# cvxopt/smcp

Hardware: AMD Instinct MI355X
Metric: Newton KKT solves/sec (higher is better)
Workload: dtype f64; 1 GPU; synth50k nested block-arrow SDP n=50000, 8073 cliques, m=100; kktsolver=chol, n=50000, cliques=8073, m=100, blkval_doubles=2493568, update_doubles=10689536, parallelism=single

## Files before the change

### smcp_amd/csrc/capi.hip

```cpp
#include <hip/hip_runtime.h>
#include <memory>
#include <unordered_map>

#include <algorithm>
#include <chrono>
#include <cstdio>
#include <cstring>
#include <map>
#include <new>
#include <string>
#include <cxxabi.h>
#include <cstdlib>
#include <atomic>
#include <thread>
#include <type_traits>
#include <vector>

#include "../../include/smcp_amd.h"
#include "constraints.hpp"
#include "context.hpp"
#include "hostpar.hpp"
#include "switches.hpp"
#include "front_generic.hip"
#include "front_mfma.hip"
// ... 322 lines not shown
      return c->D.info_host[t];
    }
  return 0;
}

constexpr int NT = 256;

template <class F>
void for_levels_up(csp_ctx* c, F f) {
  for (int64_t l = 0; l < c->S.nlev; ++l) {
    int64_t b = c->S.levptr[l], e = c->S.levptr[l + 1];
    f(c->D.levidx + b, (int)(e - b));
  }
}
template <class F>
void for_levels_down(csp_ctx* c, F f) {
  for (int64_t l = c->S.nlev - 1; l >= 0; --l) {
    int64_t b = c->S.levptr[l], e = c->S.levptr[l + 1];
    f(c->D.levidx + b, (int)(e - b));
  }
}

inline unsigned gather_parts(int namax, int64_t pairs = (int64_t)1 << 40, int ncu = 0) {
  const int base = std::max(1, std::min(64, (namax * namax) / (NT * 32)));
  if (pairs * base >= 2 * (int64_t)ncu) return (unsigned)base;
  const int cap = std::max(1, std::min(64, (namax * namax) / (NT * 2)));
  return (unsigned)std::max<int64_t>(base, std::min<int64_t>(cap, (2 * (int64_t)ncu + pairs - 1) / std::max<int64_t>(1, pairs)));
}
inline int namax_of(csp_ctx* c, const int32_t* lev) {
  const int64_t off = lev - c->D.levidx;
  const auto& lp = c->S.levptr;
  const int64_t l = std::upper_bound(lp.begin(), lp.end(), off) - lp.begin() - 1;
  return (l >= 0 && l < (int64_t)c->lev_namax.size()) ? c->lev_namax[l] : 0;
}

void gather_all(csp_ctx* c, const double* x, int64_t ldx, int nrhs, double* updbase, hipStream_t st) {
  TreeArgs a = tree_args(c);
  for_levels_down(c, [&](const int32_t* lev, int cnt) {
    a.lev = lev;
    launch(c, KID_gather_level, k_gather_level, dim3(cnt, nrhs, gather_parts(namax_of(c, lev), (int64_t)cnt * nrhs, c->D.ncu)), dim3(NT), st, a, x, ldx, updbase);
  });
}

int prepare_yaa(csp_ctx* c, const double* Y, bool need_fac, hipStream_t st, bool need_inv = false, bool allow_partial = false);
void complete_fac(csp_ctx* c, hipStream_t st);


constexpr size_t LDS_LIMIT = 160 * 1024 - 2048;

bool cache_off() {
  static int nocache = -1;
  if (nocache < 0) { const char* e = sw_str("SMCP_NOCACHE"); nocache = (e && e[0] == '1') ? 1 : 0; }
  return nocache == 1;
}

bool use_generic(const csp_ctx* c) {
  static int g = -1;
  if (g < 0) { const char* e = sw_str("SMCP_GENERIC"); g = (e && e[0] == '1') ? 1 : 0; }
  return g == 1 || (c && c->deterministic);
}

MfmaArgs mfma_args(csp_ctx* c, const double* ysc, int ymode, int nrhs) {
  MfmaArgs a;
  a.t = tree_args(c);
  a.t.lev = c->D.lev2idx;
  a.LK = c->D.lk;
  a.ysc = ysc;
  a.ymode = ymode;
  a.nnmax = a.namax = 0;
  a.nchmax = a.panmax = a.pkmax = a.plansum = 0;
  a.nrhs = nrhs;
  { static int sk = -1; if (sk < 0) { const char* e = sw_str("SMCP_SKIP"); sk = e ? atoi(e) : 0; } a.skip = sk; }
  a.dbg = (a.skip & 64) ? (unsigned long long*)(c->D.red + 768) : nullptr;
  a.lfd = c->D.lfd;
  a.dn = 0; a.dld = 0;
  a.kc_ptr = nullptr; a.kc_off = nullptr; a.kc_val = nullptr; a.kc_ids = nullptr;
  a.sp_rt = c->D.sp_rt; a.sp_mk = c->D.sp_mk;
  a.kc_stride = 0; a.kc_j0 = 0;
  a.nnmin = 0;
  a.grp_ptr = nullptr; a.grp_list = nullptr; a.chskip = nullptr; a.famt_ngrp = 0;
  a.fz_on = 0; a.fz_nat = 0; a.fz_cnn = 0; a.fz_stride = 0; a.fz_recl = 0;
  a.fz_tab = nullptr; a.fz_no = nullptr; a.fz_slot = nullptr; a.fz_ptr = nullptr; a.fz_pk = nullptr; a.fz_s = nullptr;
  a.level = 0; a.nS = 0; a.famna = a.fampan = a.fampk = a.famcna = a.famnn = a.famcnn = 0;
  return a;
}

int rhs_groups(int ncl, int nrhs, int target) {
  int g = (target + ncl - 1) / ncl;
  return std::max(1, std::min(g, nrhs));
}

template <class F>
void for_level_classes(csp_ctx* c, int64_t l, MfmaArgs a, F f, int set = 0) {
  const LevelClass& L = set ? c->sets[set].lvl[l] : c->lvl[l];
  const int32_t* base = set ? c->sets[set].lev2 + c->sets[set].off[l] : c->D.lev2idx + c->S.levptr[l];
  if (L.nI) {
    a.t.lev = base;
    a.nnmax = L.nnmaxI;
    a.namax = L.namaxI;
    a.nchmax = L.nchmaxI;
    a.panmax = L.panmaxI;
    a.pkmax = L.pkmaxI;
    a.plansum = L.plansumI;
    a.level = (int)l; a.nS = (int)L.nS; a.famna = L.famna; a.fampan = L.fampan; a.fampk = L.fampk; a.famcna = L.famcna; a.famnn = L.famnn; a.famcnn = L.famcnn;
    size_t lds = (size_t)mfma_lds_doubles(L.nnmaxI, L.namaxI) * sizeof(double);
    f(true, a, (int)L.nI, lds, lds > 48 * 1024 ? 512 : 256);
  }
  if (L.nII) {
    a.t.lev = base + L.nI;
    a.level = (int)l;
    a.nnmax = L.nnmaxII;
    a.nnmin = L.nnminII;
    a.namax = L.namaxII;
    a.nchmax = L.nchmaxII;
    f(false, a, (int)L.nII, (size_t)0, 1024);
  }
}


template <class F>
void for_all_large(csp_ctx* c, MfmaArgs a, F f) {
  if (!c->D.nII_total) return;
  a.t.lev = c->D.lev3idx + c->D.nI_total;
  a.nnmax = c->D.nnmaxII_all;
  a.namax = c->D.namaxII_all;
  f(a, (int)c->D.nII_total);
}

bool use_large() {
  static int g = -1;
  if (g < 0) { const char* e = sw_str("SMCP_LARGE"); g = (e && e[0] == '0') ? 0 : 1; }
  return g == 1;
}
inline unsigned umax1(int x) { return (unsigned)std::max(1, x); }
static int fact_threads(const MfmaArgs& am, int thr, int kind) {
  static int t[3] = {0, 0, 0};
  if (!t[0]) {
    auto rd = [](const char* n, int d, int hi) { const char* e = sw_str(n); int v = e ? atoi(e) : d; return (v >= 64 && v <= hi && !(v & 63)) ? v : d; };
    t[0] = rd("SMCP_FTHR_CHOL", 128, 1024); t[1] = rd("SMCP_FTHR_PINV", 256, 1024); t[2] = rd("SMCP_FTHR_YAA", 64, 256);
  }
  if (kind == 2 && am.nnmax <= 16 && am.namax > 32 && am.namax <= 64) {
    static int tm = 0;
    if (!tm) { const char* e = sw_str("SMCP_FTHR_YAA_MID"); tm = e ? atoi(e) : 256; if (tm < 64 || tm > 256 || (tm & 63)) tm = 256; }
    return tm;
  }
  return (am.nnmax <= 16 && am.namax <= 32) ? t[kind] : thr;
}

static bool alds_route(csp_ctx* c, const MfmaArgs& a, int cnt, int nrhs, int& nz, size_t& bytes) {
  static int alds = -1;
  if (alds < 0) { const char* e = sw_str("SMCP_ALDS"); alds = (e && e[0] == '0') ? 0 : 1; }
  const int nfmax = a.nnmax + a.namax;
  static int zenv = -1;
  if (zenv < 0) { const char* e = sw_str("SMCP_ALDS_Z"); zenv = e ? atoi(e) : 0; }
  const int64_t pairs = std::max<int64_t>(1, (int64_t)cnt * nrhs);
  nz = 1;
  if (zenv > 0) nz = zenv;
  else if (a.nchmax >= 256) nz = (int)std::max<int64_t>(1, std::min<int64_t>({(int64_t)a.nchmax / 16, (int64_t)64, (4 * (int64_t)c->D.ncu + pairs - 1) / pairs}));
  else if (nrhs >= 16 && 2 * pairs <= c->D.ncu && a.nchmax >= 32)
    nz = (int)std::max<int64_t>(1, std::min<int64_t>({(int64_t)a.nchmax / 16, (int64_t)8, (2 * (int64_t)c->D.ncu + pairs - 1) / pairs}));
  nz = std::max(1, std::min(nz, std::max(1, a.nchmax)));
  bytes = (size_t)(lf_alds_doubles(nfmax) + 4 * ((a.nchmax + nz - 1) / nz) + 2) * sizeof(double);
  if (!(alds && a.nchmax > 0 && pairs * nz >= 32 && nfmax <= LF_ALDS_MAXNF && bytes <= LDS_LIMIT)) return false;
  static bool attr = false;
  if (!attr) { attr = hipFuncSetAttribute((const void*)k_lf_assemble_lds, hipFuncAttributeMaxDynamicSharedMemorySize, 160 * 1024 - 1024) == hipSuccess; }
  return attr;
// ... 1672 lines not shown
  if (c->scal_lstar < 0) {
    int64_t ls = S.nlev;
    while (ls > 0 && c->lvl[(size_t)ls - 1].nI == 0) --ls;
    c->scal_lstar = ls;
    std::vector<int> lev_of((size_t)S.nsn, 0);
    for (int64_t l = 0; l < S.nlev; ++l)
      for (int64_t q = S.levptr[l]; q < S.levptr[l + 1]; ++q) lev_of[(size_t)S.levidx[q]] = (int)l;
    int64_t t0 = bl;
    for (int64_t k = 0; k < S.nsn; ++k) if (lev_of[(size_t)k] == S.nlev - 1) t0 = std::min<int64_t>(t0, S.blkptr[k]);
    for (int64_t k = 0; k < S.nsn; ++k) if (S.blkptr[k] >= t0 && lev_of[(size_t)k] != S.nlev - 1) { t0 = 0; break; }
    c->scal_tail0 = t0;
  }
  const int64_t lstar = c->scal_lstar;
  const bool fast = !use_generic(c) && use_large() && D.gp_tptr && !cache_off() && Fork::enabled() && scaling_overlap_on() &&
                    c->ntrial == 1 && lstar < S.nlev && (lstar > 0 || D.nI_total == 0) && D.yaa && S.updlen() > 0 && !c->verify_cache;
  if (!fast) {
    const bool li = top_li_whole(c);
    if (li) { D.lk_tag_L = D.lk_tag_Y = nullptr; D.part_valid = false; D.lk_gen++; }
    if (int rc = cholesky_impl(c, L, (void*)st, 0, li)) return rc;
    HIPCHK(hipMemcpyAsync(Y, L, sizeof(double) * bl, hipMemcpyDeviceToDevice, st));
    if (int rc = projected_inverse_impl(c, Y, (void*)st, 0, li)) return rc;
    c->D.lk_tag_L = L;
    if (flags & SCALING_FAC) { if (int rc = prepare_yaa(c, Y, true, st)) return rc; HIPCHK(end_call(c)); }
    return 0;
  }
  invalidate_tags(c, L);
  invalidate_tags(c, Y);
  HIPCHK(zero_flag(c, st));
  const int64_t last = S.nlev - 1;
  const int64_t tail0 = c->scal_tail0;
  MfmaArgs a0 = mfma_args(c, nullptr, 0, 1);
  a0.LK = nullptr;
  TreeArgs t = tree_args(c);
  int nnI = 0;
  for (const LevelClass& Lc : c->lvl) if (Lc.nI) nnI = std::max(nnI, (int)Lc.nnmaxI);
  static int cprep = -1;
  if (cprep < 0) { const char* e = sw_str("SMCP_CHOL_PREP"); cprep = (e && e[0] == '0') ? 0 : 1; }
  const bool fuse_prep = cprep && nnI <= 16;
  auto chol_small = [&](const MfmaArgs& am, int cnt, int thr) {
    const size_t lb = (size_t)mfma_lds_doubles_for(WK_CHOL, am.nnmax, am.namax) * sizeof(double);
    if (fuse_prep) launch_lds(c, KID_chol_mfma, k_chol_mfma<true, true>, dim3(cnt), dim3(fact_threads(am, thr, 0)), lb, st, am, L, D.lk);
    else launch_lds(c, KID_chol_mfma, k_chol_mfma<true>, dim3(cnt), dim3(fact_threads(am, thr, 0)), lb, st, am, L, (double*)nullptr);
  };
  auto chol_large = [&](const MfmaArgs& am, int cnt, int64_t l) { lf_chol(c, am, cnt, L, st, l == last); };
  auto chol_level = [&](int64_t l) {
    for_level_classes(c, l, a0, [&](bool lds, MfmaArgs am, int cnt, size_t bytes, int thr) {
      (void)bytes;
      if (lds) chol_small(am, cnt, thr);
      else chol_large(am, cnt, l);
    });
  };
  const ScalFam sf = scaling_fam_plan(c, a0, 0);
  if (sf.on)
    scaling_fam_up(c, sf, a0, chol_small, chol_large, [&]() {
      if (fuse_prep) launch_chol_fam<true>(c, sf, L, D.lk, st);
      else launch_chol_fam<false>(c, sf, L, (double*)nullptr, st);
    });
  for (int64_t l = sf.on ? 2 : 0; l < last; ++l) chol_level(l);
  std::unique_ptr<Fork> f0;
  if (last > 0) f0.reset(new Fork(c, st, 1));
  hipStream_t s0 = f0 ? f0->s : st;
  chol_level(last);
  if (D.nI_total && !fuse_prep) {
    TreeArgs ts = t;
    ts.lev = D.lev3idx;
    launch_lds(c, KID_prep_lk, k_prep_lk, dim3((int)D.nI_total), dim3(prep_lk_threads(nnI)), prep_lk_lds_bytes(nnI), s0, ts, (const double*)L, D.lk);
  }
  for (int64_t ll = 0; ll < last; ++ll)
    for_level_classes(c, ll, a0, [&](bool lds, MfmaArgs am, int cnt, size_t, int) { if (!lds) lf_prep(c, am, cnt, L, s0); });
  if (tail0 > 0) (void)hipMemcpyAsync(Y, L, sizeof(double) * tail0, hipMemcpyDeviceToDevice, s0);
  for_level_classes(c, last, a0, [&](bool lds, MfmaArgs am, int cnt, size_t, int) { if (!lds) lf_prep(c, am, cnt, L, st, use_top(am.nnmax + am.namax)); });
  (void)hipMemcpyAsync(Y + tail0, L + tail0, sizeof(double) * (bl - tail0), hipMemcpyDeviceToDevice, st);
  if (f0) f0->join();
  D.lk_gen++;
  D.part_valid = false;
  MfmaArgs ap = mfma_args(c, nullptr, 0, 1);
  ap.t.upd = D.yaa;
  MfmaArgs af = mfma_args(c, nullptr, 0, 1);
  const bool want_fac = (flags & SCALING_FAC) != 0;
  static int skipenv = -1;
  if (skipenv < 0) { const char* e = sw_str("SMCP_FAC_PARTIAL"); skipenv = (e && e[0] == '0') ? 0 : 1; }
  const bool skip_children = want_fac && skipenv && D.m > 0 && !D.ns && leafgram_ok(c, D.m) && c->leafgram_policy != 0;
  bool skipped = false;
  auto factor_level = [&](int64_t l, hipStream_t lds_stream, hipStream_t large_stream) {
    for_level_classes(c, l, af, [&](bool lds, MfmaArgs am, int cnt, size_t, int) {
      if (!am.namax) return;
      if (lds) {
        if (l == 0 && skip_children && am.nS > 0) { cnt -= am.nS; skipped = true; if (!cnt) return; }
        const size_t bytes = ((size_t)padld(am.namax) * am.namax + 256 + 8) * sizeof(double);
        launch_lds(c, KID_factor_yaa_lds, k_factor_yaa_lds, dim3(cnt), dim3(fact_threads(am, 256, 2)), bytes, lds_stream, am, (const double*)D.yaa, D.fac);
      } else {
        launch(c, KID_axpby, k_copy_upd_blocks, dim3(cnt, umax1(std::min(64, (am.namax * am.namax + 1023) / 1024))), dim3(256), large_stream,
               am.t, (const double*)D.yaa, D.fac);
        lf_factor_yaa(c, am, cnt, D.fac, large_stream);
      }
    });
  };
  auto pinv_small = [&](const MfmaArgs& am, int cnt, int thr) {
    launch_lds(c, KID_pinv_mfma, k_pinv_mfma<true>, dim3(cnt), dim3(fact_threads(am, thr, 1)),
               (size_t)mfma_lds_doubles_for(WK_PINV, am.nnmax, am.namax) * sizeof(double), st, am, Y);
  };
  auto pinv_large = [&](const MfmaArgs& am, int cnt, int64_t) { lf_pinv(c, am, cnt, Y, st); };
  auto pinv_level = [&](int64_t l) {
    for_level_classes(c, l, ap, [&](bool lds, MfmaArgs am, int cnt, size_t bytes, int thr) {
      (void)bytes;
      if (lds) pinv_small(am, cnt, thr);
      else pinv_large(am, cnt, l);
    });
  };
  for (int64_t l = last; l >= lstar; --l) pinv_level(l);
  bool any_large_sep = false;
  for (int64_t l = lstar; l <= last; ++l) if (c->lvl[(size_t)l].nII && c->lvl[(size_t)l].namaxII > 0) any_large_sep = true;
  std::unique_ptr<Fork> f1;
  if (want_fac && any_large_sep && lstar > 0) f1.reset(new Fork(c, st, 0));
  hipStream_t s1 = f1 ? f1->s : st;
  for (int64_t l = lstar - 1; l >= (sf.on ? 2 : 0); --l) pinv_level(l);
  if (sf.on) scaling_fam_down(c, sf, ap, pinv_small, pinv_large, [&]() { launch_pinv_fam(c, sf, ap, Y, st); });
  if (want_fac) {
    for (int64_t l = last; l >= lstar; --l) factor_level(l, s1, s1);
    for (int64_t l = lstar - 1; l >= 0; --l) factor_level(l, st, st);
  }
  if (f1) f1->join();
  D.lk_tag_L = L; D.lk_tag_Y = Y;
  D.yaa_tag = Y;
  D.fac_tag = want_fac ? Y : nullptr;
  D.fac_partial = want_fac && skipped;
  D.faci_tag = nullptr;
  if (want_fac) D.fac_gen++;
  HIPCHK(end_call(c));
  const int rc = fetch_info(c, st);
  if (rc) {
    D.lk_tag_L = D.lk_tag_Y = D.yaa_tag = D.fac_tag = D.faci_tag = nullptr;
    D.part_valid = false;
  }
  return rc;
}
int csp_cholesky_projected_inverse(csp_ctx* c, double* L, double* Y, int with_factors, void* stream) {
  if (int rc = ready(c)) return rc;
  if (!L || !Y || L == Y) return SMCP_EINVAL;
  return scaling_impl(c, L, Y, with_factors ? SCALING_FAC : 0, (hipStream_t)stream);
}

int csp_completion(csp_ctx* c, double* x, void* stream) {
  if (int rc = ready(c)) return rc;
  invalidate_tags(c, x);
  hipStream_t st = (hipStream_t)stream;
  TreeArgs a = tree_args(c);
  HIPCHK(zero_flag(c, st));
  if (!use_generic(c)) {
    prepare_yaa(c, x, true, st, true);
    MfmaArgs a0 = mfma_args(c, c->D.faci, 0, 1);
    a0.LK = nullptr;
    dim3 blk(256);
    for (int64_t l = 0; l < c->S.nlev; ++l)
      for_level_classes(c, l, a0, [&](bool lds, MfmaArgs am, int cnt, size_t bytes, int thr) {
        const size_t cb = lds ? (size_t)completion_lds_doubles(am.nnmax, am.namax) * sizeof(double) : 0;
        if (lds && cb <= LDS_LIMIT) {
          launch_lds(c, KID_completion_mfma, k_completion_mfma<true>, dim3(cnt), dim3(cb > 48 * 1024 ? 512 : 256), cb, st, am, x);
        }
        else if (lds || !use_large())
          launch_lds(c, KID_completion_mfma_hbm, k_completion_mfma<false>, dim3(cnt), dim3(lds ? 256 : thr), 0, st, am, x);
      });
    if (use_large())
      for_all_large(c, a0, [&](MfmaArgs am, int cnt) {
        const int mtA = tiles64(am.namax), ntN = tiles64(am.nnmax);
        if (am.namax) {
          launch(c, KID_lf_completion, k_lf_completion, dim3(umax1(mtA * ntN), cnt), blk, st, am, x, 0);
          launch(c, KID_lf_completion, k_lf_completion, dim3(umax1(mtA * ntN), cnt), blk, st, am, x, 1);
        }
        launch(c, KID_lf_completion, k_lf_completion, dim3(umax1(ntN * ntN), cnt), blk, st, am, x, 2);
        if (use_mid(am.nnmax))
          launch_lds(c, KID_mid_chol, k_mid_chol, dim3(cnt), dim3(1024), mid_chol_lds(am.nnmax), st, am, (double*)nullptr, (double*)nullptr, 3);
        else
// ... 350 lines not shown
```

### smcp_amd/csrc/front_mfma.hip

```cpp
#include <hip/hip_runtime.h>

namespace smcp {

typedef double d4 __attribute__((ext_vector_type(4)));

template <class FA, class FB, class FC>
__device__ inline void wg_mma(int M, int N, int Kd, FA A, FB B, FC store, bool lower_only = false, int rot = 0) {
  const int lane = threadIdx.x & 63, nw = blockDim.x >> 6;
  const int wave = ((threadIdx.x >> 6) + nw - (rot % nw)) % nw;
  const int mt = (M + 15) >> 4, nt = (N + 15) >> 4;
  const int l15 = lane & 15, kq = lane >> 4;
  for (int t = wave; t < mt * nt; t += nw) {
    const int tm = t % mt, tn = t / mt;
    if (lower_only && tm < tn) continue;
    const int m = tm * 16 + l15, nb = tn * 16 + l15;
    d4 acc = {0.0, 0.0, 0.0, 0.0};
    constexpr int KU = 2;
    for (int k0 = 0; k0 < Kd; k0 += 4 * KU) {
      double av[KU], bv[KU];
#pragma unroll
      for (int u = 0; u < KU; ++u) {
        const int k = k0 + 4 * u + kq;
        const bool kin = k < Kd;
        av[u] = (kin && m < M) ? A(m, k) : 0.0;
        bv[u] = (kin && nb < N) ? B(k, nb) : 0.0;
      }
#pragma unroll
      for (int u = 0; u < KU; ++u)
        if (k0 + 4 * u < Kd) acc = __builtin_amdgcn_mfma_f64_16x16x4f64(bv[u], av[u], acc, 0, 0, 0);
    }
#pragma unroll
    for (int r = 0; r < 4; ++r) {
      const int n = tn * 16 + kq + 4 * r;
      if (m < M && n < N) store(m, n, acc[r]);
    }
  }
}

template <int UNR, class LoadF, class UseF>
__device__ inline void batched_loop(int begin, int end, int step, LoadF load, UseF use) {
  for (int e0 = begin; e0 < end; e0 += step * UNR) {
    decltype(load(0)) v[UNR];
#pragma unroll
    for (int u = 0; u < UNR; ++u) {
      const int e = e0 + u * step;
      if (e < end) v[u] = load(e);
    }
#pragma unroll
    for (int u = 0; u < UNR; ++u) {
      const int e = e0 + u * step;
      if (e < end) use(e, v[u]);
    }
  }
}

struct MfmaArgs {
  TreeArgs t;
  const double* LK;
  const double* ysc;
  int ymode;
  int nnmax, namax;
  int nrhs;
  int nchmax, panmax, pkmax, plansum;
  int skip;
  unsigned long long* dbg;
  double* lfd;
  int dn; int64_t dld;
  const int32_t* kc_ptr; const int32_t* kc_off; const double* kc_val; const int32_t* kc_ids;
  int kc_stride, kc_j0;
  const double* sp_rt; const double* sp_mk;
  int level, nS, famna, fampan, fampk, famcna, famnn, famcnn;
  int nnmin;
  const int32_t* grp_ptr; const int32_t* grp_list; const uint8_t* chskip;
  int famt_ngrp;
  int fz_on, fz_nat, fz_cnn, fz_stride;
  int64_t fz_recl;
  const double* fz_tab; const int32_t* fz_no; const int32_t* fz_slot; const int32_t* fz_ptr; const int32_t* fz_pk; const double* fz_s;
};

__device__ __host__ inline int padld(int x) { return x | 1; }

__host__ __device__ inline int64_t mfma_lds_doubles(int nn, int na) {
  int64_t lk = padld(na), ll = padld(nn), lf = padld(nn + na);
  int64_t nnc = nn;
  return lk * nnc + ll * nnc + lk * (int64_t)na + lf * nnc + ll * nnc + lk * nnc + lk * nnc + ll * nnc + lk * (int64_t)na + 16 * 16 + 8 + (na + 2) / 2;
}

enum : int { WK_K = 1, WK_LI = 2, WK_Y = 4, WK_F = 8, WK_FNN = 16, WK_E = 32, WK_G = 64, WK_T = 128, WK_U = 256, WK_ALL = 511 };
constexpr int WK_CHOL = WK_F | WK_U;
constexpr int WK_PINV = WK_K | WK_LI | WK_E | WK_U;
constexpr int WK_DOWN0 = WK_ALL & ~(WK_Y | WK_FNN);
constexpr int WK_COMPL = WK_Y | WK_F | WK_FNN | WK_E | WK_G | WK_T;
__host__ __device__ inline int64_t mfma_lds_doubles_for(int mask, int nn, int na) {
  const int64_t lk = padld(na), ll = padld(nn), lf = padld(nn + na), nnc = nn;
  int64_t t = 0;
  if (mask & WK_K) t += lk * nnc;
  if (mask & WK_LI) t += ll * nnc;
  if (mask & WK_Y) t += lk * (int64_t)na;
  if (mask & WK_F) t += lf * nnc;
  if (mask & WK_FNN) t += ll * nnc;
  if (mask & WK_E) t += lk * nnc;
  if (mask & WK_G) t += lk * nnc;
  if (mask & WK_T) t += ll * nnc;
  if (mask & WK_U) t += lk * (int64_t)na;
  return t + 16 * 16 + 8 + (na + 2) / 2;
}
__host__ __device__ inline int64_t completion_lds_doubles(int nn, int na) {
  return mfma_lds_doubles_for(WK_COMPL, nn, na) + (nn > 16 ? 16 * 128 : 0);
}

struct Work {
  const double* K; int ldk;
  const double* Li; int ldl;
  const double* Y; int ldy;
  double* F; int ldf;
  double* Fnn; int ldn;
  double* E; int lde;
  double* G; int ldg;
  double* T; int ldt;
  double* U; int ldu;
  double* D16;
};

template <bool LDS, int MASK = WK_ALL>
__device__ inline Work make_work(const MfmaArgs& a, const CliqueDesc& d, double* smem, int k, int r) {
  Work w;
  const int nn = d.nn, na = d.na, nf = nn + na;
  if (LDS) {
    const int lk = padld(a.namax), ll = padld(a.nnmax), lf = padld(a.nnmax + a.namax);
    double* p = smem;
    w.K = p; w.ldk = lk; if (MASK & WK_K) p += (int64_t)lk * a.nnmax;
    w.Li = p; w.ldl = ll; if (MASK & WK_LI) p += (int64_t)ll * a.nnmax;
    w.Y = p; w.ldy = lk; if (MASK & WK_Y) p += (int64_t)lk * a.namax;
    w.F = p; w.ldf = lf; if (MASK & WK_F) p += (int64_t)lf * a.nnmax;
    w.Fnn = p; w.ldn = ll; if (MASK & WK_FNN) p += (int64_t)ll * a.nnmax;
    w.E = p; w.lde = lk; if (MASK & WK_E) p += (int64_t)lk * a.nnmax;
    w.G = p; w.ldg = lk; if (MASK & WK_G) p += (int64_t)lk * a.nnmax;
    w.T = p; w.ldt = ll; if (MASK & WK_T) p += (int64_t)ll * a.nnmax;
    w.U = p; w.ldu = lk; if (MASK & WK_U) p += (int64_t)lk * a.namax;
    w.D16 = p;
  } else {
    w.Li = a.LK ? a.LK + d.blk : nullptr; w.ldl = nf;
    w.K = a.LK ? a.LK + d.blk + nn : nullptr; w.ldk = nf;
    w.Y = a.ysc ? a.ysc + d.upd : nullptr; w.ldy = na;
    double* s = a.t.tmp + (int64_t)r * a.t.tmplen + a.t.tmpptr[k];
    w.Fnn = s; w.ldn = nn; s += (int64_t)nn * nn;
    w.T = s; w.ldt = nn; s += (int64_t)nn * nn;
    w.E = s; w.lde = na; s += (int64_t)na * nn;
    w.G = s; w.ldg = na; s += (int64_t)na * nn;
    w.D16 = s;
    w.F = nullptr; w.ldf = nf;
    w.U = nullptr; w.ldu = na;
  }
  return w;
}

__device__ inline void load_consts(const MfmaArgs& a, const CliqueDesc& d, const Work& w, bool needY) {
  const int nn = d.nn, na = d.na, nf = nn + na;
  if (a.LK) {
    const double* src = a.LK + d.blk;
// ... 540 lines not shown
    }
  }
}

__global__ void k_prep_lk(TreeArgs t, const double* L, double* LK) {
  const int k = t.lev ? t.lev[blockIdx.x] : blockIdx.x;
  const CliqueDesc d = t.cl[k];
  const int nn = d.nn, na = d.na, nf = nn + na;
  const double* Lk = L + d.blk;
  double* Li = LK + d.blk;
  double* Kk = Li + nn;
  __shared__ double Dinv[256];
  extern __shared__ __attribute__((aligned(16))) double S[];
  for (int e = threadIdx.x; e < nn * nn; e += blockDim.x) {
    int i = e % nn, j = e / nn;
    if (i < j) Li[i + (int64_t)j * nf] = 0.0;
  }
  for (int ib = 0; ib < nn; ib += 16) {
    const int bw = min(16, nn - ib);
    tri_inv16(Lk + ib + (int64_t)ib * nf, nf, bw, Dinv);
    for (int e = threadIdx.x; e < bw * bw; e += blockDim.x) {
      int i = e % bw, j = e / bw;
      if (i >= j) Li[(ib + i) + (int64_t)(ib + j) * nf] = Dinv[i + j * 16];
    }
    for (int c0 = 0; c0 < ib; c0 += 256) {
      const int cw = min(256, ib - c0);
      __syncthreads();
      wg_mma(bw, cw, ib - c0, [=](int m, int kk) { return Lk[(ib + m) + (int64_t)(c0 + kk) * nf]; },
             [=](int kk, int n) { return (c0 + kk >= c0 + n) ? Li[(c0 + kk) + (int64_t)(c0 + n) * nf] : 0.0; },
             [=](int m, int n, double acc) { S[m + n * 16] = acc; });
      __syncthreads();
      wg_mma(bw, cw, bw, [=](int m, int kk) { return Dinv[m + kk * 16]; },
             [=](int kk, int n) { return S[kk + n * 16]; },
             [=](int m, int n, double acc) { Li[(ib + m) + (int64_t)(c0 + n) * nf] = -acc; });
    }
    __syncthreads();
  }
  if (na) {
    wg_mma(na, nn, nn, [=](int m, int kk) { return Lk[(nn + m) + (int64_t)kk * nf]; },
           [=](int kk, int n) { return kk >= n ? Li[kk + (int64_t)n * nf] : 0.0; },
           [=](int m, int n, double acc) { Kk[m + (int64_t)n * nf] = acc; });
  }
}

template <bool LDS>
__global__ void k_pinv_mfma(MfmaArgs a, double* x) {
  extern __shared__ __attribute__((aligned(16))) double smem[];
  const int k = a.t.lev[blockIdx.x];
  const CliqueDesc d = a.t.cl[k];
  const int nn = d.nn, na = d.na, nf = nn + na;
  Work w = make_work<LDS, WK_PINV>(a, d, smem, k, 0);
  double* P = x + d.blk;
  double* UkG = a.t.upd + d.upd;
  const CliqueDesc par = a.t.cl[d.parent < 0 ? k : d.parent];
  const int32_t* rel = a.t.relidx + d.rel;
  if (LDS) {
    load_consts(a, d, w, false);
    gather_front(d, par, rel, x, a.t.upd, w.U, w.ldu, UkG);
  } else {
    w.U = UkG;
    gather_front(d, par, rel, x, a.t.upd, UkG, na, nullptr);
  }
  __syncthreads();
  const Work v = w;
  wg_mma(na, nn, na, [=](int m, int kk) { return m >= kk ? v.U[m + kk * v.ldu] : v.U[kk + m * v.ldu]; },
         [=](int kk, int n) { return v.K[kk + n * v.ldk]; },
         [=](int m, int n, double acc) { v.E[m + n * v.lde] = acc; });
  __syncthreads();
  wg_mma(nn, nn, nn + na,
         [=](int m, int kk) { return kk < nn ? v.Li[kk + m * v.ldl] : v.K[(kk - nn) + m * v.ldk]; },
         [=](int kk, int n) { return kk < nn ? v.Li[kk + n * v.ldl] : v.E[(kk - nn) + n * v.lde]; },
         [=](int m, int n, double acc) { if (m >= n) P[m + (int64_t)n * nf] = acc; });
  for (int e = threadIdx.x; e < na * nn; e += blockDim.x) {
    int i = e % na, j = e / na;
    P[nn + i + (int64_t)j * nf] = -v.E[i + j * v.lde];
  }
}




__global__ void __launch_bounds__(256) k_factor_yaa_lds(MfmaArgs a, const double* yaa, double* fac) {
  extern __shared__ __attribute__((aligned(16))) double smem[];
  const int k = a.t.lev[blockIdx.x];
  const CliqueDesc d = a.t.cl[k];
  const int na = d.na;
  if (!na) return;
  const int ld = padld(a.namax);
  double* const M = smem;
  double* const D16 = smem + (int64_t)ld * a.namax;
  const double* src = yaa + d.upd;
  double* dst = fac + d.upd;
  batched_loop<8>(threadIdx.x, na * na, blockDim.x, [=](int e) { return (e % na) >= (e / na) ? src[e] : 0.0; },
                  [=](int e, double v) { M[(e % na) + (e / na) * ld] = v; });
  for (int jb = 0; jb < na; jb += 16) {
    const int bw = min(16, na - jb);
    int f = potrf_inv16(M + jb + jb * ld, ld, bw, D16);
    if (f) { if (threadIdx.x == 0) atomicCAS(info_of(a.t, k), 0, info_val(a.t, k)); return; }
    const int mrem = na - jb - bw;
    if (mrem > 0) {
      double* Pj = M + (jb + bw) + jb * ld;
      wg_mma(mrem, bw, bw, [=](int m, int kk) { return Pj[m + kk * ld]; },
             [=](int kk, int n) { return D16[n + kk * 16]; },
             [=](int m, int n, double acc) { Pj[m + n * ld] = acc; });
      __syncthreads();
      double* Tr = M + (jb + bw) + (jb + bw) * ld;
      wg_mma(mrem, mrem, bw, [=](int m, int kk) { return Pj[m + kk * ld]; },
             [=](int kk, int n) { return Pj[n + kk * ld]; },
             [=](int m, int n, double acc) { if (m >= n) Tr[m + n * ld] -= acc; }, true);
      __syncthreads();
    }
  }
  for (int e = threadIdx.x; e < na * na; e += blockDim.x) {
    int i = e % na, j = e / na;
    if (i >= j) dst[e] = M[i + j * ld];
  }
}

struct PadL {
  int NN, NA, ldn, lda;
  int oK, oBD, oY, oFnn, oFan, oE, oG, oQ, oT, oU, oInt, total;
  int iCh, iPan, iOut, iTgt;
};
__host__ __device__ inline PadL pad_layout(int nnmax, int namax, int nchmax = 0, int panmax = 0, int pkmax = 0,
                                           int plansum = 0) {
  PadL L;
  L.NN = (nnmax + 15) & ~15;
  L.NA = (namax + 15) & ~15;
  L.ldn = L.NN + 1;
  L.lda = L.NA + 1;
  int o = 0;
  L.oK = o; o += L.lda * L.NN;
  L.oBD = o; o += L.ldn * L.NN;
  L.oY = o; o += L.lda * L.NA;
  L.oFnn = o; o += L.ldn * L.NN;
  L.oFan = o; o += L.lda * L.NN;
  L.oE = o; o += L.lda * L.NN;
  if (L.NN == 16) { L.oG = L.oFan; L.oQ = L.oE; } else { L.oG = o; o += L.lda * L.NN; L.oQ = L.oFan; }
  L.oT = o; o += L.ldn * L.NN;
  L.oU = o; if (nchmax > 0) o += L.lda * L.NA;
  L.oInt = o;
  L.iCh = 0;
  L.iPan = 4 * nchmax;
  L.iOut = L.iPan + panmax;
  L.iTgt = L.iOut + pkmax;
  o += (L.iTgt + plansum + 3) / 2;
  L.total = o + 2;
  return L;
}

__device__ inline void lds_barrier() { asm volatile("s_waitcnt lgkmcnt(0)\n\ts_barrier" ::: "memory"); }

__device__ inline void mma_run(d4& acc, const double* pa, int sa, const double* pb, int sb, int ks) {
#pragma unroll 4
  for (int s = 0; s < ks; ++s) {
    const double av = *pa, bv = *pb;
    pa += sa;
    pb += sb;
    acc = __builtin_amdgcn_mfma_f64_16x16x4f64(bv, av, acc, 0, 0, 0);
  }
}

__global__ void __launch_bounds__(512) k_hess_up_pad(MfmaArgs a, double* u, int64_t ldu) {
  extern __shared__ __attribute__((aligned(16))) double smem[];
  const int k = a.t.lev[blockIdx.x];
  const CliqueDesc d = a.t.cl[k];
  const int nn = d.nn, na = d.na, nf = nn + na;
// ... 522 lines not shown
```

### smcp_amd/csrc/front_top.hip

```cpp
#pragma once

namespace smcp {

constexpr int TOP_MAXT = 13;
constexpr int TOP_MAXROWS = 16 * TOP_MAXT;
constexpr int TOP_TW = 15;
constexpr int TOP_SLOTS = (TOP_MAXT * (TOP_MAXT + 1) / 2 + TOP_TW - 1) / TOP_TW;

#define TOP_WAVE_FENCE() do { __builtin_amdgcn_fence(__ATOMIC_RELEASE, "wavefront"); __builtin_amdgcn_wave_barrier(); \
                              __builtin_amdgcn_fence(__ATOMIC_ACQUIRE, "wavefront"); } while (0)

template <bool INV>
__global__ void __launch_bounds__(1024) k_top_chol(MfmaArgs a, double* x, double* LK) {
  __shared__ __attribute__((aligned(16))) double s_d[256];
  __shared__ __attribute__((aligned(16))) double s_inv[TOP_MAXT * 256];
  __shared__ __attribute__((aligned(16))) double s_pan[TOP_MAXT * 256];
  __shared__ int s_fail;
  const int k = a.t.lev[blockIdx.x];
  if (*info_of(a.t, k)) return;
  const CliqueDesc d = a.t.cl[k];
  const int nn = d.nn, na = d.na, nf = nn + na;
  if (nf > TOP_MAXROWS) return;
  const int tid = threadIdx.x, lane = tid & 63, wave = __builtin_amdgcn_readfirstlane(tid >> 6), l15 = lane & 15, kq = lane >> 4;
  const int nt = (nf + 15) >> 4, nct = (nn + 15) >> 4, ntile = nt * (nt + 1) / 2;
  double* const P = x + d.blk;
  if (tid == 0) s_fail = 0;
  __syncthreads();

  if (wave == TOP_TW) {
    for (int r = 0; r < nct; ++r) {
      __syncthreads();
      const bool ok = wave_potrf_inv16(s_d, 16, min(16, nn - 16 * r), s_inv + 256 * r);
      if (!ok && lane == 0) s_fail = 1;
      __syncthreads();
      if (!ok) { if (lane == 0) atomicCAS(info_of(a.t, k), 0, info_val(a.t, k)); return; }
      __syncthreads();
    }
  } else {
    const double* const U = a.t.upd + d.upd;
    unsigned vo[4], vu[4];
#pragma unroll
    for (int q = 0; q < 4; ++q) { vo[q] = l15 + (kq + 4 * q) * nf; vu[q] = l15 + (kq + 4 * q) * na; }
    int ti[TOP_SLOTS], tj[TOP_SLOTS];
    bool valid[TOP_SLOTS];
    d4 T[TOP_SLOTS];
#pragma unroll
    for (int s = 0; s < TOP_SLOTS; ++s) {
      const int t = TOP_TW * s + wave;
      int i = 0;
      while ((i + 1) * (i + 2) / 2 <= t) ++i;
      ti[s] = i; tj[s] = t - i * (i + 1) / 2;
      valid[s] = t < ntile;
#pragma unroll
      for (int q = 0; q < 4; ++q) {
        const int row = 16 * i + l15, col = 16 * tj[s] + kq + 4 * q;
        const bool ok = valid[s] && row < nf && col <= row;
        const double* src = !ok ? P : (col < nn ? &(P + (16 * i + 16 * tj[s] * nf))[vo[q]] : &(U + ((16 * i - nn) + (16 * tj[s] - nn) * na))[vu[q]]);
        const double v = *src;
        T[s][q] = ok ? v : 0.0;
      }
      __builtin_amdgcn_sched_barrier(0);
    }
    auto update = [&](d4& t, int i, int j) {
      const double* Pi = s_pan + 256 * i;
      const double* Pj = s_pan + 256 * j;
#pragma unroll
      for (int q = 0; q < 4; ++q) t = __builtin_amdgcn_mfma_f64_16x16x4f64(Pj[l15 + 16 * (4 * q + kq)], -Pi[l15 + 16 * (4 * q + kq)], t, 0, 0, 0);
      __builtin_amdgcn_sched_barrier(0);
    };
    for (int r = 0; r < nct; ++r) {
      const int bw = min(16, nn - 16 * r);
      const bool part = bw < 16;
#pragma unroll
      for (int s = 0; s < TOP_SLOTS; ++s)
        if (valid[s] && ti[s] == r && tj[s] == r) {
          if (r > 0) update(T[s], r, r);
#pragma unroll
          for (int q = 0; q < 4; ++q) s_d[l15 + 16 * (kq + 4 * q)] = T[s][q];
        }
      __syncthreads();
      if (r > 0) {
#pragma unroll
        for (int s = 0; s < TOP_SLOTS; ++s)
          if (valid[s] && tj[s] >= r && ti[s] > r) update(T[s], ti[s], tj[s]);
      }
      __syncthreads();
      if (s_fail) return;
      int l15b = l15, kqb = kq;
      asm volatile("" : "+v"(l15b), "+v"(kqb));
      const double* Xr = s_inv + 256 * r;
#pragma unroll
      for (int s = 0; s < TOP_SLOTS; ++s) {
        if (!valid[s] || tj[s] != r) continue;
        const bool diag = ti[s] == r;
        if (diag) {
#pragma unroll
          for (int q = 0; q < 4; ++q) {
            const int col = kqb + 4 * q;
            if (l15b < bw && col <= l15b) {
              T[s][q] = s_d[l15b + 16 * col];
              (P + (16 * r + 16 * r * nf))[vo[q]] = T[s][q];
            }
          }
          if (!part) continue;
        }
        d4 p = {0.0, 0.0, 0.0, 0.0};
#pragma unroll
        for (int q = 0; q < 4; ++q) {
          const double av = (!part || 4 * q + kqb < bw) ? T[s][q] : 0.0;
          p = __builtin_amdgcn_mfma_f64_16x16x4f64(Xr[l15b + 16 * (4 * q + kqb)], av, p, 0, 0, 0);
        }
        double* Ps = s_pan + 256 * ti[s];
        const int row = 16 * ti[s] + l15b;
        const bool below = !diag || l15b >= bw;
#pragma unroll
        for (int q = 0; q < 4; ++q) {
          const int col = kqb + 4 * q;
          const double v = below ? p[q] : 0.0;
          Ps[l15b + 16 * col] = v;
          if (below && col < bw) {
            T[s][q] = v;
            if (row < nf) (P + (16 * ti[s] + 16 * r * nf))[vo[q]] = v;
          }
        }
        __builtin_amdgcn_sched_barrier(0);
      }
      __syncthreads();
    }
    if (na > 0) {
      const int j0 = (nn & 15) ? nct - 1 : nct;
      double* UP = a.t.updp + d.updp;
      int l15f = l15, kqf = kq;
      asm volatile("" : "+v"(l15f), "+v"(kqf));
#pragma unroll
      for (int s = 0; s < TOP_SLOTS; ++s) {
        if (!valid[s] || tj[s] < j0) continue;
        update(T[s], ti[s], tj[s]);
#pragma unroll
        for (int q = 0; q < 4; ++q) {
          const int row = 16 * ti[s] + l15f, col = 16 * tj[s] + kqf + 4 * q;
          if (row < nf && col >= nn && col <= row) UP[pk_idx(row - nn, col - nn, na)] = T[s][q];
        }
      }
    }
  }
  if (!INV) return;
  for (int c = wave; c < nct; c += 16) {
    const int cw = min(16, nn - 16 * c);
    double* Xc = LK + d.blk + (int64_t)(16 * c) * nf;
    const bool mok = l15 < cw;
    for (int e = lane; e < 16 * c * cw; e += 64) Xc[e % (16 * c) + (int64_t)(e / (16 * c)) * nf] = 0.0;
    d4 z;
#pragma unroll
    for (int q = 0; q < 4; ++q) {
      const int n = kq + 4 * q;
      z[q] = n >= l15 ? s_inv[256 * c + n + 16 * l15] : 0.0;
      if (mok && n < cw) Xc[(16 * c + n) + (int64_t)l15 * nf] = z[q];
    }
    const double* __restrict__ Lp = P;
    double* __restrict__ Xw = Xc;
    const bool lastok = 16 * (nct - 1) + l15 < nn;
    const unsigned lo = l15 + kq * nf, lo_last = (lastok ? l15 : 0) + kq * nf;
    d4 S[TOP_MAXT - 1];
#pragma unroll
    for (int j = 0; j < TOP_MAXT - 1; ++j) S[j] = d4{0.0, 0.0, 0.0, 0.0};
#pragma unroll
    for (int ks = 0; ks < TOP_MAXT - 1; ++ks) {
      const int kt = c + ks;
      if (kt + 1 < nct) {
#pragma unroll
        for (int j = ks; j < TOP_MAXT - 1; ++j) {
          const int r = min(c + 1 + j, nct - 1);
          const bool last = r == nct - 1;
          const bool rok = c + 1 + j < nct && (!last || lastok);
#pragma unroll
          for (int q = 0; q < 4; ++q) {
            const double b0 = (Lp + (16 * r + (16 * kt + 4 * q) * nf))[last ? lo_last : lo];
            S[j] = __builtin_amdgcn_mfma_f64_16x16x4f64(rok ? b0 : 0.0, z[q], S[j], 0, 0, 0);
          }
        }
        const int r = kt + 1, rw = min(16, nn - 16 * r);
        d4 zn = {0.0, 0.0, 0.0, 0.0};
#pragma unroll
        for (int q = 0; q < 4; ++q) zn = __builtin_amdgcn_mfma_f64_16x16x4f64(s_inv[256 * r + l15 + 16 * (4 * q + kq)], S[ks][q], zn, 0, 0, 0);
#pragma unroll
        for (int q = 0; q < 4; ++q) {
          const int n = kq + 4 * q;
          z[q] = -zn[q];
          if (mok && n < rw) Xw[(16 * r + n) + (int64_t)l15 * nf] = z[q];
        }
      }
    }
  }
}
#undef TOP_WAVE_FENCE

}
```

Baseline: 373.4 KKT solves/s.

## Fold level-0 yaa factor into level-1 launch and pipeline top Cholesky diagonal

Merges the small level-0 LDS yaa factorization launch into the level-1 launch by appending level-0 cliques to the grid through a split index, which removes one kernel launch. In k_top_chol the diagonal-block update now runs on the dedicated potrf wave using a double-buffered s_d, and the next diagonal tile is staged early, so one __syncthreads per panel step is dropped. The inverse phase assigns one wave per tile column and batches panel loads ahead of the MFMAs for more memory-level parallelism. Optional timestamp instrumentation is added behind SMCP_STAMPS. The risks are load imbalance from mixing cliques of different sizes in one grid and higher register pressure from the batched loads.

```diff
diff --git a/smcp_amd/csrc/capi.hip b/smcp_amd/csrc/capi.hip
--- a/smcp_amd/csrc/capi.hip
+++ b/smcp_amd/csrc/capi.hip
@@ -428,6 +428,7 @@
   a.fz_on = 0; a.fz_nat = 0; a.fz_cnn = 0; a.fz_stride = 0; a.fz_recl = 0;
   a.fz_tab = nullptr; a.fz_no = nullptr; a.fz_slot = nullptr; a.fz_ptr = nullptr; a.fz_pk = nullptr; a.fz_s = nullptr;
   a.level = 0; a.nS = 0; a.famna = a.fampan = a.fampk = a.famcna = a.famnn = a.famcnn = 0;
+  a.lev_b = nullptr; a.lev_split = 0;
   return a;
 }
 
@@ -2266,13 +2267,22 @@
   if (skipenv < 0) { const char* e = sw_str("SMCP_FAC_PARTIAL"); skipenv = (e && e[0] == '0') ? 0 : 1; }
   const bool skip_children = want_fac && skipenv && D.m > 0 && !D.ns && leafgram_ok(c, D.m) && c->leafgram_policy != 0;
   bool skipped = false;
+  YaaFold fold{false, 0, 0, 0};
+  if (want_fac && lstar >= 2) {
+    const LevelClass &L0 = c->lvl[0], &L1 = c->lvl[1];
+    const int64_t rest0 = L0.nI - ((skip_children && L0.nS > 0) ? L0.nS : 0);
+    fold = yaa_fold_plan(L1.nI, L1.nI ? L1.namaxI : 0, rest0, L0.nI ? L0.namaxI : 0);
+  }
   auto factor_level = [&](int64_t l, hipStream_t lds_stream, hipStream_t large_stream) {
     for_level_classes(c, l, af, [&](bool lds, MfmaArgs am, int cnt, size_t, int) {
       if (!am.namax) return;
       if (lds) {
         if (l == 0 && skip_children && am.nS > 0) { cnt -= am.nS; skipped = true; if (!cnt) return; }
+        if (l == 0 && fold.on) return;
+        const int thr = fact_threads(am, 256, 2);
+        if (l == 1 && fold.on) { am.lev_b = D.lev2idx + S.levptr[0]; am.lev_split = fold.split; cnt = fold.grid; }
         const size_t bytes = ((size_t)padld(am.namax) * am.namax + 256 + 8) * sizeof(double);
-        launch_lds(c, KID_factor_yaa_lds, k_factor_yaa_lds, dim3(cnt), dim3(fact_threads(am, 256, 2)), bytes, lds_stream, am, (const double*)D.yaa, D.fac);
+        launch_lds(c, KID_factor_yaa_lds, k_factor_yaa_lds, dim3(cnt), dim3(thr), bytes, lds_stream, am, (const double*)D.yaa, D.fac);
       } else {
         launch(c, KID_axpby, k_copy_upd_blocks, dim3(cnt, umax1(std::min(64, (am.namax * am.namax + 1023) / 1024))), dim3(256), large_stream,
                am.t, (const double*)D.yaa, D.fac);
diff --git a/smcp_amd/csrc/front_mfma.hip b/smcp_amd/csrc/front_mfma.hip
--- a/smcp_amd/csrc/front_mfma.hip
+++ b/smcp_amd/csrc/front_mfma.hip
@@ -1,4 +1,5 @@
 #include <hip/hip_runtime.h>
+#include "yaa_fold.hpp"
 
 namespace smcp {
 
@@ -76,6 +77,7 @@
   int fz_on, fz_nat, fz_cnn, fz_stride;
   int64_t fz_recl;
   const double* fz_tab; const int32_t* fz_no; const int32_t* fz_slot; const int32_t* fz_ptr; const int32_t* fz_pk; const double* fz_s;
+  const int32_t* lev_b; int lev_split;
 };
 
 __device__ __host__ inline int padld(int x) { return x | 1; }
@@ -782,7 +784,7 @@
 
 __global__ void __launch_bounds__(256) k_factor_yaa_lds(MfmaArgs a, const double* yaa, double* fac) {
   extern __shared__ __attribute__((aligned(16))) double smem[];
-  const int k = a.t.lev[blockIdx.x];
+  const int k = yaa_fold_clique(a.t.lev, a.lev_b, a.lev_split, blockIdx.x);
   const CliqueDesc d = a.t.cl[k];
   const int na = d.na;
   if (!na) return;
diff --git a/smcp_amd/csrc/front_top.hip b/smcp_amd/csrc/front_top.hip
--- a/smcp_amd/csrc/front_top.hip
+++ b/smcp_amd/csrc/front_top.hip
@@ -6,16 +6,29 @@
 constexpr int TOP_MAXROWS = 16 * TOP_MAXT;
 constexpr int TOP_TW = 15;
 constexpr int TOP_SLOTS = (TOP_MAXT * (TOP_MAXT + 1) / 2 + TOP_TW - 1) / TOP_TW;
+constexpr int TOP_INVB = 4;
+__host__ __device__ constexpr int top_inv_batch(int ks, int j) { return (ks == 0 && j >= TOP_MAXT - 3) ? 1 : (ks < 3 ? 2 : (ks < 6 ? 3 : 4)); }
 
 #define TOP_WAVE_FENCE() do { __builtin_amdgcn_fence(__ATOMIC_RELEASE, "wavefront"); __builtin_amdgcn_wave_barrier(); \
                               __builtin_amdgcn_fence(__ATOMIC_ACQUIRE, "wavefront"); } while (0)
+#ifdef SMCP_STAMPS
+#define TOP_STAMP(i) do { if (stamp) { const unsigned long long t_ = wall_clock64(); s_tph[i] += t_ - s_tm[threadIdx.x ? 1 : 0]; s_tm[threadIdx.x ? 1 : 0] = t_; } } while (0)
+#else
+#define TOP_STAMP(i) do { } while (0)
+#endif
 
 template <bool INV>
 __global__ void __launch_bounds__(1024) k_top_chol(MfmaArgs a, double* x, double* LK) {
-  __shared__ __attribute__((aligned(16))) double s_d[256];
+  __shared__ __attribute__((aligned(16))) double s_d[2 * 256];
   __shared__ __attribute__((aligned(16))) double s_inv[TOP_MAXT * 256];
   __shared__ __attribute__((aligned(16))) double s_pan[TOP_MAXT * 256];
   __shared__ int s_fail;
+#ifdef SMCP_STAMPS
+  __shared__ unsigned long long s_tph[16], s_tm[2];
+  const bool stamp = a.dbg && blockIdx.x == 0 && (threadIdx.x == 0 || threadIdx.x == 64 * TOP_TW);
+  if (stamp) s_tm[threadIdx.x ? 1 : 0] = wall_clock64();
+  if (threadIdx.x < 16) s_tph[threadIdx.x] = 0;
+#endif
   const int k = a.t.lev[blockIdx.x];
   if (*info_of(a.t, k)) return;
   const CliqueDesc d = a.t.cl[k];
@@ -28,13 +41,29 @@
   __syncthreads();
 
   if (wave == TOP_TW) {
+    __syncthreads();
+    TOP_STAMP(8);
     for (int r = 0; r < nct; ++r) {
-      __syncthreads();
-      const bool ok = wave_potrf_inv16(s_d, 16, min(16, nn - 16 * r), s_inv + 256 * r);
+      double* const Dr = s_d + 256 * (r & 1);
+      if (r > 0) {
+        const double* Pr = s_pan + 256 * r;
+        d4 t;
+#pragma unroll
+        for (int q = 0; q < 4; ++q) t[q] = Dr[l15 + 16 * (kq + 4 * q)];
+#pragma unroll
+        for (int q = 0; q < 4; ++q) t = __builtin_amdgcn_mfma_f64_16x16x4f64(Pr[l15 + 16 * (4 * q + kq)], -Pr[l15 + 16 * (4 * q + kq)], t, 0, 0, 0);
+#pragma unroll
+        for (int q = 0; q < 4; ++q) Dr[l15 + 16 * (kq + 4 * q)] = t[q];
+        TOP_WAVE_FENCE();
+      }
+      TOP_STAMP(10);
+      const bool ok = wave_potrf_inv16(Dr, 16, min(16, nn - 16 * r), s_inv + 256 * r);
+      TOP_STAMP(9);
       if (!ok && lane == 0) s_fail = 1;
       __syncthreads();
       if (!ok) { if (lane == 0) atomicCAS(info_of(a.t, k), 0, info_val(a.t, k)); return; }
       __syncthreads();
+      TOP_STAMP(8);
     }
   } else {
     const double* const U = a.t.upd + d.upd;
@@ -68,23 +97,28 @@
       for (int q = 0; q < 4; ++q) t = __builtin_amdgcn_mfma_f64_16x16x4f64(Pj[l15 + 16 * (4 * q + kq)], -Pi[l15 + 16 * (4 * q + kq)], t, 0, 0, 0);
       __builtin_amdgcn_sched_barrier(0);
     };
+    if (wave == 0) {
+#pragma unroll
+      for (int q = 0; q < 4; ++q) s_d[l15 + 16 * (kq + 4 * q)] = T[0][q];
+    }
+    __syncthreads();
+    TOP_STAMP(0);
     for (int r = 0; r < nct; ++r) {
       const int bw = min(16, nn - 16 * r);
       const bool part = bw < 16;
 #pragma unroll
-      for (int s = 0; s < TOP_SLOTS; ++s)
-        if (valid[s] && ti[s] == r && tj[s] == r) {
-          if (r > 0) update(T[s], r, r);
-#pragma unroll
-          for (int q = 0; q < 4; ++q) s_d[l15 + 16 * (kq + 4 * q)] = T[s][q];
-        }
-      __syncthreads();
-      if (r > 0) {
-#pragma unroll
-        for (int s = 0; s < TOP_SLOTS; ++s)
-          if (valid[s] && tj[s] >= r && ti[s] > r) update(T[s], ti[s], tj[s]);
-      }
-      __syncthreads();
+      for (int s = 0; s < TOP_SLOTS; ++s) {
+        if (!valid[s] || tj[s] < r) continue;
+        if (r > 0 && (ti[s] > r || part)) update(T[s], ti[s], tj[s]);
+        if (ti[s] == r + 1 && tj[s] == r + 1 && r + 1 < nct) {
+          double* Dn = s_d + 256 * ((r + 1) & 1);
+#pragma unroll
+          for (int q = 0; q < 4; ++q) Dn[l15 + 16 * (kq + 4 * q)] = T[s][q];
+        }
+      }
+      TOP_STAMP(2);
+      __syncthreads();
+      TOP_STAMP(3);
       if (s_fail) return;
       int l15b = l15, kqb = kq;
       asm volatile("" : "+v"(l15b), "+v"(kqb));
@@ -98,7 +132,7 @@
           for (int q = 0; q < 4; ++q) {
             const int col = kqb + 4 * q;
             if (l15b < bw && col <= l15b) {
-              T[s][q] = s_d[l15b + 16 * col];
+              T[s][q] = (s_d + 256 * (r & 1))[l15b + 16 * col];
               (P + (16 * r + 16 * r * nf))[vo[q]] = T[s][q];
             }
           }
@@ -125,7 +159,9 @@
         }
         __builtin_amdgcn_sched_barrier(0);
       }
-      __syncthreads();
+      TOP_STAMP(4);
+      __syncthreads();
+      TOP_STAMP(5);
     }
     if (na > 0) {
       const int j0 = (nn & 15) ? nct - 1 : nct;
@@ -144,18 +180,30 @@
       }
     }
   }
+  TOP_STAMP(6);
+#ifdef SMCP_STAMPS
+  if (!INV && stamp) {
+    const int o = threadIdx.x ? 8 : 0;
+    for (int i = o; i < o + 8; ++i) atomicAdd(a.dbg + 16 + i, s_tph[i]);
+    if (!threadIdx.x) atomicAdd(a.dbg + 16 + 13, 1ull);
+  }
+#endif
   if (!INV) return;
-  for (int c = wave; c < nct; c += 16) {
+  static_assert(TOP_MAXT <= TOP_TW + 1, "one wave per tile column");
+  if (wave < nct) {
+    const int c = wave;
     const int cw = min(16, nn - 16 * c);
     double* Xc = LK + d.blk + (int64_t)(16 * c) * nf;
     const bool mok = l15 < cw;
-    for (int e = lane; e < 16 * c * cw; e += 64) Xc[e % (16 * c) + (int64_t)(e / (16 * c)) * nf] = 0.0;
+    for (int m = 0; m < cw; ++m)
+      for (int i = lane; i < 16 * c; i += 64) (Xc + m * nf)[i] = 0.0;
+    const unsigned xo = kq + l15 * nf;
     d4 z;
 #pragma unroll
     for (int q = 0; q < 4; ++q) {
       const int n = kq + 4 * q;
       z[q] = n >= l15 ? s_inv[256 * c + n + 16 * l15] : 0.0;
-      if (mok && n < cw) Xc[(16 * c + n) + (int64_t)l15 * nf] = z[q];
+      if (mok && n < cw) (Xc + (16 * c + 4 * q))[xo] = z[q];
     }
     const double* __restrict__ Lp = P;
     double* __restrict__ Xw = Xc;
@@ -169,15 +217,27 @@
       const int kt = c + ks;
       if (kt + 1 < nct) {
 #pragma unroll
-        for (int j = ks; j < TOP_MAXT - 1; ++j) {
-          const int r = min(c + 1 + j, nct - 1);
-          const bool last = r == nct - 1;
-          const bool rok = c + 1 + j < nct && (!last || lastok);
-#pragma unroll
-          for (int q = 0; q < 4; ++q) {
-            const double b0 = (Lp + (16 * r + (16 * kt + 4 * q) * nf))[last ? lo_last : lo];
-            S[j] = __builtin_amdgcn_mfma_f64_16x16x4f64(rok ? b0 : 0.0, z[q], S[j], 0, 0, 0);
-          }
+        for (int j = ks; j < TOP_MAXT - 1; j += top_inv_batch(ks, j)) {
+          const int nb = top_inv_batch(ks, j);
+          double b0[TOP_INVB][4];
+#pragma unroll
+          for (int u = 0; u < TOP_INVB; ++u) {
+            if (u >= nb || j + u >= TOP_MAXT - 1) continue;
+            const int r = min(c + 1 + j + u, nct - 1);
+            const bool last = r == nct - 1;
+#pragma unroll
+            for (int q = 0; q < 4; ++q) b0[u][q] = (Lp + (16 * r + (16 * kt + 4 * q) * nf))[last ? lo_last : lo];
+          }
+          __builtin_amdgcn_sched_barrier(0);
+#pragma unroll
+          for (int u = 0; u < TOP_INVB; ++u) {
+            if (u >= nb || j + u >= TOP_MAXT - 1) continue;
+            const bool last = min(c + 1 + j + u, nct - 1) == nct - 1;
+            const bool rok = c + 1 + j + u < nct && (!last || lastok);
+#pragma unroll
+            for (int q = 0; q < 4; ++q) S[j + u] = __builtin_amdgcn_mfma_f64_16x16x4f64(rok ? b0[u][q] : 0.0, z[q], S[j + u], 0, 0, 0);
+          }
+          __builtin_amdgcn_sched_barrier(0);
         }
         const int r = kt + 1, rw = min(16, nn - 16 * r);
         d4 zn = {0.0, 0.0, 0.0, 0.0};
@@ -187,12 +247,22 @@
         for (int q = 0; q < 4; ++q) {
           const int n = kq + 4 * q;
           z[q] = -zn[q];
-          if (mok && n < rw) Xw[(16 * r + n) + (int64_t)l15 * nf] = z[q];
-        }
-      }
-    }
-  }
+          if (mok && n < rw) (Xw + (16 * r + 4 * q))[xo] = z[q];
+        }
+      }
+    }
+  }
+#ifdef SMCP_STAMPS
+  if (stamp) {
+    __builtin_amdgcn_s_waitcnt(0);
+    TOP_STAMP(7);
+    const int o = threadIdx.x ? 8 : 0;
+    for (int i = o; i < o + 8; ++i) atomicAdd(a.dbg + i, s_tph[i]);
+    if (!threadIdx.x) atomicAdd(a.dbg + 13, 1ull);
+  }
+#endif
 }
 #undef TOP_WAVE_FENCE
+#undef TOP_STAMP
 
 }
diff --git a/smcp_amd/csrc/yaa_fold.hpp b/smcp_amd/csrc/yaa_fold.hpp
--- /dev/null
+++ b/smcp_amd/csrc/yaa_fold.hpp
@@ -0,0 +1,35 @@
+#pragma once
+#include <cstdint>
+
+#if defined(__HIPCC__)
+#define SMCP_FOLD_HD __host__ __device__
+#else
+#define SMCP_FOLD_HD
+#endif
+
+namespace smcp {
+
+struct YaaFold {
+  bool on;
+  int grid;
+  int split;
+  int namax;
+};
+
+inline YaaFold yaa_fold_plan(int64_t cnt_a, int namax_a, int64_t cnt_b, int namax_b) {
+  YaaFold f{false, (int)cnt_a, 0, namax_a};
+  if (cnt_a <= 0 || cnt_b <= 0 || namax_a <= 0 || namax_b <= 0) return f;
+  if (namax_b > namax_a) return f;
+  if (cnt_b * 8 > cnt_a) return f;
+  if (cnt_a + cnt_b > INT32_MAX) return f;
+  f.on = true;
+  f.grid = (int)(cnt_a + cnt_b);
+  f.split = (int)cnt_a;
+  return f;
+}
+
+SMCP_FOLD_HD inline int32_t yaa_fold_clique(const int32_t* lev, const int32_t* lev_b, int split, int b) {
+  return (lev_b && split > 0 && b >= split) ? lev_b[b - split] : lev[b];
+}
+
+}
```

Measured after the change: 376.2 KKT solves/s, median of 6. Within noise of the previous version (+0.7%).
